# Soldann/MORB_SLAM

Measured on AMD Instinct MI355X. Metric: stereo frames/sec ORB extract+match (752x480, 1200 feat = BASELINE configs[1]), higher is better.
Workload: dtype u8; 1 GPU; BASELINE configs[1]: EuRoC-shaped stereo 752x480, 1200 feat: ORBextractor x2 + ComputeStereoMatches + ComputeBoW (synthetic k=10 L=6 vocabulary) + SearchByBoW vs previous frame; steps_in_flight=2, extract_streams=1, parallelism=frames dealt round-robin over 1 GPU(s)

## Files before the change

### morb_slam_amd/csrc/handles.h

```cpp
#pragma once
#include <cstdint>
#include <vector>

#include "common.h"
#include "hip_owned.h"

struct morb_matcher {
  int device = 0;
  morb::Stream stream;
  morb::DeviceGrow sortA;
  morb::DeviceGrow bin;
  morb::DeviceGrow sad;
  morb::DeviceGrow stereoRec;
  morb::DeviceGrow candKeys;
  morb::DeviceGrow candCount;
  morb::DeviceGrow evictJ;
  morb::DeviceGrow evictB;
  morb::DeviceGrow pairTables;
  morb::DeviceGrow newPointPairs;
  morb::DeviceGrow queries;
  morb::DeviceGrow queryCount;
  morb::DeviceGrow kfdbPair;
  morb::DeviceGrow kfdbList;
  morb::DeviceGrow scratch;
  struct ConstCopy { morb::DeviceArray<> d; std::vector<uint8_t> host; unsigned long long used = 0; };
  struct ConstSlot { ConstCopy way[4]; unsigned long long clock = 0; };
  enum ConstTable {
    kThresholdsPinhole = 0,
    kThresholdsKB8 = 1,
    kRigLastFrame = 2,
  };
  ConstSlot consts[4];
  std::vector<morb::DeviceArray<>> retired;
};

struct morb_optimizer {
  int device = 0;
  morb::Stream stream;
  morb::Stream side;
  morb::Event evFork, evJoin;
  morb::DeviceGrow work;
  morb::DeviceGrow spill;
  morb::DeviceGrow mlpnpCorr;
  morb::DeviceGrow twoViewCorr;
  morb::PinnedGrow stage;
  morb::PinnedArray<int> lmWords;
  int exactOrder = 1;
// ... 31 lines not shown
```

### morb_slam_amd/csrc/matcher.hip

```cpp
#include <hip/hip_runtime.h>

#include <algorithm>
#include <cstdlib>
#include <cstring>
#include <memory>
#include <vector>

#include "common.h"
#include "internal_abi.h"
#include "wave.h"
#include "extractor_internal.h"

using namespace morb;

namespace {

constexpr int TH_HIGH = 100, TH_LOW = 50, HISTO_LENGTH = 30;

struct Desc { uint32_t w[8]; };

__device__ __forceinline__ Desc load_desc(const uint8_t* p) {
  Desc d;
  const uint4* q = reinterpret_cast<const uint4*>(p);
  const uint4 a = q[0], b = q[1];
  d.w[0] = a.x; d.w[1] = a.y; d.w[2] = a.z; d.w[3] = a.w;
// ... 522 lines not shown
#pragma unroll
      for (int j = 0; j < CH; ++j) tc[j] = *reinterpret_cast<const uint2*>(nd + (size_t)min(cb + j, c0 + nc - 1) * 32);
#pragma unroll
      for (int j = 0; j < CH; ++j) {
        const int dd = quad_sum(__popc(d.x ^ tc[j].x) + __popc(d.y ^ tc[j].y));
        if (dd < bestd) { bestd = dd; best = min(cb + j, c0 + nc - 1); }
      }
    }
    final_id = best;
    if (level == nid_level) nid = final_id;
  } while (firstChild[final_id] >= 0);
  if (sub == 0) { wordId[o] = final_id; nodeId[o] = nid; }
}

__global__ __launch_bounds__(1024) void k_bow_sort(const int* __restrict__ node, const int* __restrict__ count, int cap,
                                                   int P, unsigned long long* __restrict__ sorted) {
  extern __shared__ unsigned long long skeys[];
  const int img = blockIdx.x, tid = threadIdx.x, NT = blockDim.x;
  const int n = count[img];
  if (n == 0) {
    for (int i = tid; i < cap; i += NT) sorted[(size_t)img * cap + i] = ~0ull;
    return;
  }
  for (int i = tid; i < P; i += NT) {
    unsigned long long k = ~0ull;
    if (i < n) {
      const int nd = node[(size_t)img * cap + i];
      if (nd >= 0) k = ((unsigned long long)(unsigned)nd << 32) | (unsigned)i;
    }
    skeys[i] = k;
  }
  __syncthreads();
  const bool onePass = P / 2 <= NT;
  for (int k = 2; k <= P; k <<= 1)
    for (int j = k >> 1; j > 0; j >>= 1) {
      for (int l = tid; l < P / 2; l += NT) {
        const int i = ((l & ~(j - 1)) << 1) | (l & (j - 1)), ixj = i | j;
        const unsigned long long a = skeys[i], b = skeys[ixj];
        const bool up = (i & k) == 0;
        if ((a > b) == up) { skeys[i] = b; skeys[ixj] = a; }
      }
      const int jn = j > 1 ? j >> 1 : k;
      if (onePass && jn < 64 && j < 64) { __builtin_amdgcn_fence(__ATOMIC_SEQ_CST, "wavefront"); __builtin_amdgcn_wave_barrier(); }
      else __syncthreads();
    }
  for (int i = tid; i < cap; i += NT) sorted[(size_t)img * cap + i] = i < P ? skeys[i] : ~0ull;
}

#ifdef MORB_FAST_TIMING
__device__ unsigned long long g_bowTrace[16384 * 4];
#define BOW_MARK(k) do { if (lane == 0 && bw_ < 16384) g_bowTrace[bw_ * 4 + (k)] = wall_clock64(); } while (0)
#else
#define BOW_MARK(k)
#endif
constexpr int BM_NB = 25;
constexpr int BM_FJ = 4;
__device__ __forceinline__ unsigned wave_min_u32(unsigned v) { return morbwave::min_u32(v); }
__global__ __launch_bounds__(256) void k_bow_match(const unsigned long long* __restrict__ sortedKF,
                                                   const unsigned long long* __restrict__ sortedF,
                                                   const int* __restrict__ nKFv, const int* __restrict__ nFv, int cap,
                                                   const uint8_t* __restrict__ descKF, const uint8_t* __restrict__ hasMP,
                                                   const morb_keypoint* __restrict__ kpsKF,
                                                   const uint8_t* __restrict__ descF, const morb_keypoint* __restrict__ kpsF,
                                                   const int* __restrict__ kfImg, const int* __restrict__ fImg,
                                                   float nnratio, int* __restrict__ matchF, int* __restrict__ binF,
                                                   const int* __restrict__ nLeftv,
                                                   const uint8_t* __restrict__ hasMP2, const int* __restrict__ nValidv,
                                                   int* __restrict__ matched2) {
  extern __shared__ __align__(16) unsigned long long bowLds[];
#ifdef MORB_FAST_TIMING
  const int bw_ = (blockIdx.y * gridDim.x + blockIdx.x) * 4 + (threadIdx.x >> 6);
  if ((threadIdx.x & 63) == 0 && bw_ < 16384) g_bowTrace[bw_ * 4] = wall_clock64();
#endif
  unsigned long long* sk = bowLds;
  unsigned long long* sf = bowLds + cap;
  const int pair = blockIdx.y, tid = threadIdx.x, lane = tid & 63, wv = tid >> 6;
  const int ik = kfImg[pair], jf = fImg[pair];
  const int nKF = nKFv[ik], nF = nFv[jf];
  const bool fish = nLeftv != nullptr && nLeftv[pair] >= 0;
  const int nLeft = fish ? nLeftv[pair] : 0x7fffffff;
  const bool kfkf = hasMP2 != nullptr;
  const int nValid1 = (kfkf && nValidv) ? nValidv[ik] : 0x7fffffff, nValid2 = (kfkf && nValidv) ? nValidv[jf] : 0x7fffffff;
  const int thLow = kfkf ? TH_LOW - 1 : TH_LOW;
  {
    const unsigned long long* gk = sortedKF + (size_t)ik * cap;
    const unsigned long long* gf = sortedF + (size_t)jf * cap;
    for (int i0 = 0; i0 < cap; i0 += 256 * 4) {
      unsigned long long a[4], b[4];
#pragma unroll
      for (int k = 0; k < 4; ++k) {
        const int i = i0 + k * 256 + tid;
        a[k] = i < nKF ? gk[i] : ~0ull;
        b[k] = i < nF ? gf[i] : ~0ull;
      }
#pragma unroll
      for (int k = 0; k < 4; ++k) {
        const int i = i0 + k * 256 + tid;
        if (i < nKF) sk[i] = a[k];
        if (i < nF) sf[i] = b[k];
      }
    }
  }
  __syncthreads();
  BOW_MARK(1);
  uint16_t* starts = reinterpret_cast<uint16_t*>(sf + cap);
  __shared__ int wcnt[4];
  const uint64_t ltm = lane == 0 ? 0ull : (~0ull >> (64 - lane));
  int nStarts = 0;
  for (int i0 = 0; i0 < nKF; i0 += 256) {
    const int i = i0 + tid;
    bool st = false;
    if (i < nKF) {
      const unsigned long long k = sk[i];
      st = k != ~0ull && (i == 0 || (unsigned)(sk[i - 1] >> 32) != (unsigned)(k >> 32));
    }
    const uint64_t m = __ballot(st);
    if (lane == 0) wcnt[wv] = __popcll(m);
    __syncthreads();
    int off = nStarts;
    for (int w = 0; w < wv; ++w) off += wcnt[w];
    if (st) starts[off + __popcll(m & ltm)] = (uint16_t)i;
    nStarts += wcnt[0] + wcnt[1] + wcnt[2] + wcnt[3];
    __syncthreads();
  }
  const int G = gridDim.x * 4, g = blockIdx.x * 4 + wv;
  BOW_MARK(2);
  int* mF = matchF + (size_t)pair * cap;
  int* bF = binF + (size_t)pair * cap;
  const float factor = 1.0f / HISTO_LENGTH;
  for (int o = g; o < nStarts; o += G) {
    const int p = starts[o];
    const unsigned node = (unsigned)(sk[p] >> 32);
    int lo = 0, hi = nF;
    const unsigned long long target = (unsigned long long)node << 32;
    while (lo < hi) {
      const int mid = (lo + hi) >> 1;
      if (sf[mid] < target) lo = mid + 1; else hi = mid;
    }
    const int fBeg = lo;
    int nFs = 0;
    bool more = false;
#pragma unroll
    for (int j = 0; j < BM_FJ; ++j) {
      const int s = fBeg + j * 64 + lane;
      const uint64_t mm = __ballot(s < nF && (unsigned)(sf[s] >> 32) == node);
      nFs += __popcll(mm);
      more = mm == ~0ull;
      if (mm != ~0ull) break;
    }
    if (nFs == 0) continue;
    if (!more) {
      const int nJ = (nFs + 63) >> 6;
      int idxF[BM_FJ], myMatch[BM_FJ], myBin[BM_FJ];
      Desc dF[BM_FJ];
      float angF[BM_FJ];
#pragma unroll
      for (int j = 0; j < BM_FJ; ++j) {
        idxF[j] = 0; myMatch[j] = -1; myBin[j] = 0; angF[j] = 0.f; dF[j] = Desc{};
        if (j < nJ && j * 64 + lane < nFs) {
          idxF[j] = (int)(sf[fBeg + j * 64 + lane] & 0xFFFFFFFFu);
          dF[j] = load_desc(descF + ((size_t)jf * cap + idxF[j]) * 32);
          angF[j] = kpsF[(size_t)jf * cap + idxF[j]].angle;
          if (kfkf && (!hasMP2[(size_t)jf * cap + idxF[j]] || idxF[j] >= nValid2)) myMatch[j] = -2;
        }
      }
      for (int q0 = p; q0 < nKF; q0 += 64) {
        const uint64_t mK = __ballot(q0 + lane < nKF && (unsigned)(sk[q0 + lane] >> 32) == node);
        const int nKs = mK == ~0ull ? 64 : (int)__builtin_ctzll(~mK);
        if (nKs == 0) break;
        int idxK = 0, has = 0;
        Desc dK = {};
        float angK = 0.f;
        if (lane < nKs) {
          idxK = (int)(sk[q0 + lane] & 0xFFFFFFFFu);
          has = hasMP[(size_t)ik * cap + idxK] && idxK < nValid1;
          dK = load_desc(descKF + ((size_t)ik * cap + idxK) * 32);
          angK = kpsKF[(size_t)ik * cap + idxK].angle;
        }
        for (int q = 0; q < nKs; ++q) {
          if (!__builtin_amdgcn_readlane(has, q)) continue;
          Desc dk;
#pragma unroll
          for (int w = 0; w < 8; ++w) dk.w[w] = (uint32_t)__builtin_amdgcn_readlane((int)dK.w[w], q);
          unsigned a1 = ~0u, a2 = ~0u;
          unsigned b1 = ~0u;
#pragma unroll
          for (int j = 0; j < BM_FJ; ++j)
            if (j < nJ && j * 64 + lane < nFs && myMatch[j] == -1) {
              const unsigned key = ((unsigned)hamming(dk, dF[j]) << 16) | (unsigned)idxF[j];
              if (idxF[j] < nLeft) { if (key < a1) { a2 = a1; a1 = key; } else if (key < a2) a2 = key; }
              else if (key < b1) b1 = key;
            }
          const unsigned k1 = wave_min_u32(a1);
          const unsigned k2 = wave_min_u32(a1 == k1 ? a2 : a1);
          const unsigned r1 = fish ? wave_min_u32(b1) : ~0u;
          const int bestDist1 = k1 == ~0u ? 256 : (int)(k1 >> 16);
          const int bestDist2 = k2 == ~0u ? 256 : (int)(k2 >> 16);
          const int bestDist1R = r1 == ~0u ? 256 : (int)(r1 >> 16);
          if (bestDist1 <= thLow) {
            const int realIdxKF = __builtin_amdgcn_readlane(idxK, q);
            const float aK = __int_as_float(__builtin_amdgcn_readlane(__float_as_int(angK), q));
            const bool takeL = (float)bestDist1 < nnratio * (float)bestDist2;
            const bool takeR = bestDist1R <= TH_LOW;
            const int wantIdx = (takeL && a1 == k1) ? (int)(k1 & 0xFFFFu) : -1;
            const int wantIdxR = (takeR && b1 == r1 && r1 != ~0u) ? (int)(r1 & 0xFFFFu) : -1;
#pragma unroll
            for (int j = 0; j < BM_FJ; ++j)
              if (j < nJ && j * 64 + lane < nFs && myMatch[j] == -1 && (idxF[j] == wantIdx || idxF[j] == wantIdxR)) {
                float rot = aK - angF[j];
                if (rot < 0.0f) rot += 360.0f;
                int bin = (int)roundf(rot * factor);
                if (bin == HISTO_LENGTH) bin = 0;
                myMatch[j] = realIdxKF; myBin[j] = bin;
              }
          }
        }
        if (nKs < 64) break;
      }
#pragma unroll
      for (int j = 0; j < BM_FJ; ++j)
        if (j < nJ && j * 64 + lane < nFs && myMatch[j] >= 0) {
          if (kfkf) { mF[myMatch[j]] = idxF[j]; bF[myMatch[j]] = myBin[j]; }
          else { mF[idxF[j]] = myMatch[j]; bF[idxF[j]] = myBin[j]; }
        }
      continue;
    }
    int fEnd = fBeg;
    while (fEnd < nF && (unsigned)(sf[fEnd] >> 32) == node) ++fEnd;
    for (int q = p; q < nKF; ++q) {
      const unsigned long long kq = sk[q];
      if (kq == ~0ull || (unsigned)(kq >> 32) != node) break;
      const int realIdxKF = (int)(kq & 0xFFFFFFFFu);
      if (!hasMP[(size_t)ik * cap + realIdxKF] || realIdxKF >= nValid1) continue;
      const Desc dKF = load_desc(descKF + ((size_t)ik * cap + realIdxKF) * 32);
      unsigned long long k1 = ~0ull, k2 = ~0ull, r1 = ~0ull, r2 = ~0ull;
      for (int s0 = fBeg; s0 < fEnd; s0 += 64) {
        const int s = s0 + lane;
        if (s < fEnd) {
          const int realIdxF = (int)(sf[s] & 0xFFFFFFFFu);
          const bool cand = kfkf ? (hasMP2[(size_t)jf * cap + realIdxF] && realIdxF < nValid2 && !matched2[(size_t)pair * cap + realIdxF])
                                 : (mF[realIdxF] < 0);
          if (cand) {
            const int d = hamming(dKF, load_desc(descF + ((size_t)jf * cap + realIdxF) * 32));
            const unsigned long long key = ((unsigned long long)d << 32) | (unsigned)realIdxF;
            const bool left = realIdxF < nLeft;
            unsigned long long t1 = left ? k1 : r1, t2 = left ? k2 : r2;
            top2_insert(t1, t2, key);
            k1 = left ? t1 : k1; k2 = left ? t2 : k2; r1 = left ? r1 : t1; r2 = left ? r2 : t2;
          }
        }
      }
      wave_top2(k1, k2);
      if (fish) wave_top2(r1, r2);
      const int bestDist1 = k1 == ~0ull ? 256 : (int)(k1 >> 32);
      const int bestDist2 = k2 == ~0ull ? 256 : (int)(k2 >> 32);
      const int bestDist1R = r1 == ~0ull ? 256 : (int)(r1 >> 32);
      if (bestDist1 <= thLow) {
        const float aK = kpsKF[(size_t)ik * cap + realIdxKF].angle;
        const bool takeL = (float)bestDist1 < nnratio * (float)bestDist2, takeR = bestDist1R <= TH_LOW;
        if (lane == 0) {
          if (takeL) {
            const int bestIdxF = (int)(k1 & 0xFFFFFFFFu);
            float rot = aK - kpsF[(size_t)jf * cap + bestIdxF].angle;
            if (rot < 0.0f) rot += 360.0f;
            int bin = (int)roundf(rot * factor);
            if (bin == HISTO_LENGTH) bin = 0;
            if (kfkf) { mF[realIdxKF] = bestIdxF; bF[realIdxKF] = bin; matched2[(size_t)pair * cap + bestIdxF] = 1; }
            else { mF[bestIdxF] = realIdxKF; bF[bestIdxF] = bin; }
          }
          if (takeR) {
            const int bestIdxFR = (int)(r1 & 0xFFFFFFFFu);
            float rot = aK - kpsF[(size_t)jf * cap + bestIdxFR].angle;
            if (rot < 0.0f) rot += 360.0f;
            int bin = (int)roundf(rot * factor);
            if (bin == HISTO_LENGTH) bin = 0;
            mF[bestIdxFR] = realIdxKF; bF[bestIdxFR] = bin;
          }
        }
        __builtin_amdgcn_fence(__ATOMIC_SEQ_CST, "workgroup");
        __builtin_amdgcn_wave_barrier();
      }
    }
  }
#ifdef MORB_FAST_TIMING
  BOW_MARK(3);
#endif
}

__global__ __launch_bounds__(64) void k_distinctive(const int* __restrict__ start, const uint8_t* __restrict__ desc,
                                                    int* __restrict__ bestIdx) {
  const int mp = blockIdx.x, lane = threadIdx.x;
  const int s0 = start[mp], N = start[mp + 1] - s0;
  if (N <= 0) { if (lane == 0) bestIdx[mp] = -1; return; }
  const uint8_t* D = desc + (size_t)s0 * 32;
  const int k = (N - 1) >> 1;
  unsigned best = ~0u;
  for (int i0 = 0; i0 < N; i0 += 64) {
// ... 17 lines not shown
}

__device__ void three_maxima(const int* cnt, int L, int& ind1, int& ind2, int& ind3) {
  int max1 = 0, max2 = 0, max3 = 0;
  ind1 = ind2 = ind3 = -1;
  for (int i = 0; i < L; i++) {
    const int s = cnt[i];
    if (s > max1) { max3 = max2; max2 = max1; max1 = s; ind3 = ind2; ind2 = ind1; ind1 = i; }
    else if (s > max2) { max3 = max2; max2 = s; ind3 = ind2; ind2 = i; }
    else if (s > max3) { max3 = s; ind3 = i; }
  }
  if (max2 < 0.1f * (float)max1) { ind2 = -1; ind3 = -1; }
  else if (max3 < 0.1f * (float)max1) { ind3 = -1; }
}

__global__ __launch_bounds__(256) void k_rot_filter(const int* __restrict__ nFv, const int* __restrict__ fImg, int cap,
                                                    int checkOri, int* __restrict__ matchF, const int* __restrict__ binF,
                                                    int* __restrict__ nmatches) {
  __shared__ int hist[HISTO_LENGTH];
  __shared__ int keep[3];
  __shared__ int total;
  const int pair = blockIdx.x, tid = threadIdx.x;
  const int nF = nFv[fImg[pair]];
  int* mF = matchF + (size_t)pair * cap;
  const int* bF = binF + (size_t)pair * cap;
  if (tid < HISTO_LENGTH) hist[tid] = 0;
  if (tid == 0) total = 0;
  __syncthreads();
  for (int i = tid; i < nF; i += 256)
    if (mF[i] >= 0) { atomicAdd(&total, 1); if (checkOri) atomicAdd(&hist[bF[i]], 1); }
  __syncthreads();
  if (checkOri) {
    if (tid == 0) three_maxima(hist, HISTO_LENGTH, keep[0], keep[1], keep[2]);
    __syncthreads();
    for (int i = tid; i < nF; i += 256)
      if (mF[i] >= 0) {
        const int b = bF[i];
        if (b != keep[0] && b != keep[1] && b != keep[2]) { mF[i] = -1; atomicSub(&total, 1); }
      }
    __syncthreads();
  }
  if (tid == 0) nmatches[pair] = total;
}

__global__ void k_fill_i32(int* p, size_t n, int v) {
  const size_t i = (size_t)blockIdx.x * 256 + threadIdx.x;
  if (i < n) p[i] = v;
}

}

extern "C" {

int morb_matcher_create(morb_matcher** out, int device) {
  MORB_REQUIRE(out, MORB_ERR_INVALID, "out is NULL");
  *out = nullptr;
  int ndev = 0;
// ... 35 lines not shown
    if (c.way[w].used < c.way[victim].used) victim = w;
  }
  morb_matcher::ConstCopy& k = c.way[victim];
  morb::DeviceArray<> fresh;
  MORB_HIP_CHECK(fresh.alloc(bytes));
  if (k.d) m->retired.push_back(std::move(k.d));
  k.d = std::move(fresh);
  k.host.assign((const uint8_t*)host, (const uint8_t*)host + bytes);
  k.used = ++c.clock;
  hipStream_t st = stream_or_own(m, stream);
  MORB_HIP_CHECK(hipMemcpyAsync(k.d, k.host.data(), bytes, hipMemcpyHostToDevice, st));
  MORB_HIP_CHECK(hipStreamSynchronize(st));
  *d_out = k.d;
  return MORB_OK;
}
int morb_bow_sort_images(morb_matcher* m, int nimg, const int* d_node, const int* d_count, int cap, unsigned long long** d_sorted,
                         void* stream) {
  int P = 1;
  while (P < cap) P <<= 1;
  MORB_REQUIRE((size_t)P * 8 <= 160 * 1024, MORB_ERR_UNSUPPORTED, "too many features per frame for the LDS sort");
  hipStream_t st = stream_or_own(m, stream);
  unsigned long long* sortA = nullptr;
  int rc = grow(m->sortA, (size_t)nimg * cap, &sortA);
  if (rc != MORB_OK) return rc;
  MORB_HIP_CHECK(hipFuncSetAttribute(reinterpret_cast<const void*>(k_bow_sort), hipFuncAttributeMaxDynamicSharedMemorySize, P * 8));
  hipLaunchKernelGGL(k_bow_sort, dim3(nimg), dim3(P / 2 < 64 ? 64 : P / 2 > 1024 ? 1024 : P / 2), (size_t)P * 8, st, d_node, d_count, cap, P, sortA);
  *d_sorted = sortA;
  return MORB_OK;
}

size_t morb_feature_slab_bytes(int S, int cap) {
  if (S <= 0 || cap <= 0) return 0;
  return (size_t)S * cap * (sizeof(morb_keypoint) + 32 + sizeof(int)) + (size_t)S * sizeof(int);
}
namespace {
__global__ __launch_bounds__(256) void k_slab_copy(int S, int cap, const int* __restrict__ rowIdx, uint32_t* kps, uint32_t* desc, uint32_t* node, int* count,
                                                   uint32_t* slab, int dir) {
  const int f = blockIdx.x, which = blockIdx.y;
  const int row = rowIdx ? rowIdx[f] : f;
  const size_t wK = (size_t)cap * 7, wD = (size_t)cap * 8, wN = (size_t)cap;
  uint32_t* sK = slab; uint32_t* sD = sK + (size_t)S * wK; uint32_t* sN = sD + (size_t)S * wD; uint32_t* sC = sN + (size_t)S * wN;
// ... 192 lines not shown
  MORB_REQUIRE(v, MORB_ERR_INVALID, "NULL vocabulary");
  if (weight) memcpy(weight, v->weight.data(), v->weight.size() * sizeof(double));
  if (scoring) *scoring = v->scoring;
  if (weighting) *weighting = v->weighting;
  return MORB_OK;
}

static int search_by_bow_impl(morb_matcher* m, int npairs, const int* d_kfImg, const int* d_fImg, int nimg,
                              const morb_keypoint* d_kps, const uint8_t* d_desc, const int* d_node, const int* d_count,
                              const uint8_t* d_hasMP, int cap, float nnratio, int checkOri, int* d_matchF,
                              int* d_nmatches, const int* d_nLeft, void* stream, const uint8_t* d_hasMP2 = nullptr,
                              const int* d_nValid = nullptr) {
  MORB_REQUIRE(m && d_kfImg && d_fImg && d_kps && d_desc && d_node && d_count && d_hasMP && d_matchF && d_nmatches,
               MORB_ERR_INVALID, "NULL argument");
  MORB_REQUIRE(npairs > 0 && nimg > 0 && cap > 0, MORB_ERR_INVALID, "bad sizes");
  int P = 1;
  while (P < cap) P <<= 1;
  MORB_REQUIRE((size_t)P * 8 <= 160 * 1024, MORB_ERR_UNSUPPORTED, "too many features per frame for the LDS sort");
  MORB_ENTER(st, m, stream);
  unsigned long long* sortA = nullptr;
  int* bin = nullptr;
  int rc = grow(m->sortA, (size_t)nimg * cap, &sortA);
  if (rc != MORB_OK) return rc;
  rc = grow(m->bin, (size_t)npairs * cap, &bin);
  if (rc != MORB_OK) return rc;
  MORB_HIP_CHECK(hipFuncSetAttribute(reinterpret_cast<const void*>(k_bow_sort), hipFuncAttributeMaxDynamicSharedMemorySize, P * 8));
  hipLaunchKernelGGL(k_bow_sort, dim3(nimg), dim3(P / 2 < 64 ? 64 : P / 2 > 1024 ? 1024 : P / 2), (size_t)P * 8, st, d_node, d_count, cap, P, sortA);
  const size_t nm = (size_t)npairs * cap;
  hipLaunchKernelGGL(k_fill_i32, dim3((unsigned)((nm + 255) / 256)), dim3(256), 0, st, d_matchF, nm, -1);
  int* matched2 = nullptr;
  if (d_hasMP2) {
    rc = grow(m->scratch, nm, &matched2);
    if (rc != MORB_OK) return rc;
    hipLaunchKernelGGL(k_fill_i32, dim3((unsigned)((nm + 255) / 256)), dim3(256), 0, st, matched2, nm, 0);
  }
  MORB_REQUIRE(cap < 65536 && (size_t)cap * 18 <= 160 * 1024, MORB_ERR_UNSUPPORTED, "too many features per frame for the LDS-resident node tables");
  MORB_HIP_CHECK(hipFuncSetAttribute(reinterpret_cast<const void*>(k_bow_match), hipFuncAttributeMaxDynamicSharedMemorySize, (int)((size_t)cap * 18)));
  hipLaunchKernelGGL(k_bow_match, dim3(BM_NB, npairs), dim3(256), (size_t)cap * 18, st, sortA, sortA, d_count, d_count,
                     cap, d_desc, d_hasMP, d_kps, d_desc, d_kps, d_kfImg, d_fImg, nnratio, d_matchF, bin, d_nLeft, d_hasMP2,
                     d_nValid, matched2);
  hipLaunchKernelGGL(k_rot_filter, dim3(npairs), dim3(256), 0, st, d_count, d_hasMP2 ? d_kfImg : d_fImg, cap, checkOri, d_matchF,
                     bin, d_nmatches);
  MORB_HIP_CHECK(hipGetLastError());
  return MORB_OK;
}

int morb_search_by_bow_batch(morb_matcher* m, int npairs, const int* d_kfImg, const int* d_fImg, int nimg,
                             const morb_keypoint* d_kps, const uint8_t* d_desc, const int* d_node, const int* d_count,
                             const uint8_t* d_hasMP, int cap, float nnratio, int checkOri, int* d_matchF,
                             int* d_nmatches, void* stream) {
  return search_by_bow_impl(m, npairs, d_kfImg, d_fImg, nimg, d_kps, d_desc, d_node, d_count, d_hasMP, cap, nnratio, checkOri,
                            d_matchF, d_nmatches, nullptr, stream);
}
// ... 37 lines not shown
```

Before: 140,100 frames/s.

## Precompute BoW node segments in sort kernel and add per-pair match kernel

The BoW sort kernel now also emits per-image segment tables (node id, first index, length), so the match kernel no longer rebuilds segment starts in every block of every pair. A new single-block-per-pair match kernel with LDS-resident 16-bit index tables, dynamic segment dealing and a fused rotation filter is added, but it is only chosen when npairs is at least 256 or an env var forces it. The change also caches the dynamic-LDS attribute calls and stops padding the sorted arrays out to cap. The cost is an extra segment pass inside the sort kernel and more code paths to keep correct.

```diff
diff --git a/morb_slam_amd/csrc/bow_segments.h b/morb_slam_amd/csrc/bow_segments.h
--- /dev/null
+++ b/morb_slam_amd/csrc/bow_segments.h
@@ -0,0 +1,50 @@
+#pragma once
+#include <cstdint>
+
+#if defined(__HIPCC__)
+#define BOWSEG_HD __host__ __device__ __forceinline__
+#else
+#define BOWSEG_HD inline
+#endif
+
+namespace morbseg {
+
+constexpr unsigned long long NO_WORD = ~0ull;
+
+BOWSEG_HD bool segment_starts(const unsigned long long* keys, int i) {
+  const unsigned long long k = keys[i];
+  return k != NO_WORD && (i == 0 || (uint32_t)(keys[i - 1] >> 32) != (uint32_t)(k >> 32));
+}
+
+BOWSEG_HD void segment_entry(const unsigned long long* keys, int n, int first, uint32_t* node, uint32_t* range) {
+  const uint32_t nd = (uint32_t)(keys[first] >> 32);
+  const unsigned long long last = ((unsigned long long)nd << 32) | 0xFFFFFFFFull;
+  int lo = first + 1, hi = n;
+  while (lo < hi) {
+    const int mid = (lo + hi) >> 1;
+    if (keys[mid] <= last) lo = mid + 1; else hi = mid;
+  }
+  *node = nd;
+  *range = (uint32_t)first | ((uint32_t)(lo - first) << 16);
+}
+
+BOWSEG_HD int segment_first(uint32_t range) { return (int)(range & 0xFFFFu); }
+BOWSEG_HD int segment_length(uint32_t range) { return (int)(range >> 16); }
+
+BOWSEG_HD int segment_find(const uint32_t* table, int nSeg, uint32_t node) {
+  int lo = 0, hi = nSeg;
+  while (lo < hi) {
+    const int mid = (lo + hi) >> 1;
+    if (table[2 * mid] < node) lo = mid + 1; else hi = mid;
+  }
+  return lo < nSeg && table[2 * lo] == node ? lo : -1;
+}
+
+inline int bow_segments_serial(const unsigned long long* keys, int n, uint32_t* table) {
+  int nSeg = 0;
+  for (int i = 0; i < n; ++i)
+    if (segment_starts(keys, i)) { segment_entry(keys, n, i, &table[2 * nSeg], &table[2 * nSeg + 1]); ++nSeg; }
+  return nSeg;
+}
+
+}
diff --git a/morb_slam_amd/csrc/handles.h b/morb_slam_amd/csrc/handles.h
--- a/morb_slam_amd/csrc/handles.h
+++ b/morb_slam_amd/csrc/handles.h
@@ -9,6 +9,7 @@
   int device = 0;
   morb::Stream stream;
   morb::DeviceGrow sortA;
+  morb::DeviceGrow bowSeg;
   morb::DeviceGrow bin;
   morb::DeviceGrow sad;
   morb::DeviceGrow stereoRec;
@@ -31,6 +32,7 @@
     kRigLastFrame = 2,
   };
   ConstSlot consts[4];
+  int bowSortLds = 0, bowMatchLds = 0, bowPairLds = 0;
   std::vector<morb::DeviceArray<>> retired;
 };
 
diff --git a/morb_slam_amd/csrc/matcher.hip b/morb_slam_amd/csrc/matcher.hip
--- a/morb_slam_amd/csrc/matcher.hip
+++ b/morb_slam_amd/csrc/matcher.hip
@@ -9,6 +9,7 @@
 #include "common.h"
 #include "internal_abi.h"
 #include "wave.h"
+#include "bow_segments.h"
 #include "extractor_internal.h"
 
 using namespace morb;
@@ -561,12 +562,14 @@
 }
 
 __global__ __launch_bounds__(1024) void k_bow_sort(const int* __restrict__ node, const int* __restrict__ count, int cap,
-                                                   int P, unsigned long long* __restrict__ sorted) {
+                                                   int P, unsigned long long* __restrict__ sorted,
+                                                   uint2* __restrict__ seg, int* __restrict__ segCount) {
   extern __shared__ unsigned long long skeys[];
+  __shared__ int wcnt[16];
   const int img = blockIdx.x, tid = threadIdx.x, NT = blockDim.x;
-  const int n = count[img];
-  if (n == 0) {
-    for (int i = tid; i < cap; i += NT) sorted[(size_t)img * cap + i] = ~0ull;
+  const int n = min(count[img], cap);
+  if (n <= 0) {
+    if (segCount && tid == 0) segCount[img] = 0;
     return;
   }
   for (int i = tid; i < P; i += NT) {
@@ -591,7 +594,30 @@
       if (onePass && jn < 64 && j < 64) { __builtin_amdgcn_fence(__ATOMIC_SEQ_CST, "wavefront"); __builtin_amdgcn_wave_barrier(); }
       else __syncthreads();
     }
-  for (int i = tid; i < cap; i += NT) sorted[(size_t)img * cap + i] = i < P ? skeys[i] : ~0ull;
+  __syncthreads();
+  for (int i = tid; i < n; i += NT) sorted[(size_t)img * cap + i] = skeys[i];
+  if (!seg) return;
+  const int lane = tid & 63, wv = tid >> 6, nW = NT >> 6;
+  const uint64_t ltm = lane == 0 ? 0ull : (~0ull >> (64 - lane));
+  uint2* sg = seg + (size_t)img * cap;
+  int nSeg = 0;
+  for (int i0 = 0; i0 < n; i0 += NT) {
+    const int i = i0 + tid;
+    const bool st = i < n && morbseg::segment_starts(skeys, i);
+    const uint64_t m = __ballot(st);
+    if (lane == 0) wcnt[wv] = __popcll(m);
+    __syncthreads();
+    int off = nSeg, all = 0;
+    for (int w = 0; w < nW; ++w) { const int c = wcnt[w]; all += c; off += w < wv ? c : 0; }
+    if (st) {
+      uint2 e;
+      morbseg::segment_entry(skeys, n, i, &e.x, &e.y);
+      sg[off + __popcll(m & ltm)] = e;
+    }
+    nSeg += all;
+    __syncthreads();
+  }
+  if (tid == 0) segCount[img] = nSeg;
 }
 
 #ifdef MORB_FAST_TIMING
@@ -602,9 +628,190 @@
 #endif
 constexpr int BM_NB = 25;
 constexpr int BM_FJ = 4;
+#ifndef MORB_BM_PAIR_WAVES
+#define MORB_BM_PAIR_WAVES 8
+#endif
+constexpr int BM_PAIR_WAVES = MORB_BM_PAIR_WAVES;
+constexpr int BM_PAIR_LONG = 16;
+constexpr int BM_PAIR_FROM = 256;
+constexpr int BM_PAIR_LDS = 13;
 __device__ __forceinline__ unsigned wave_min_u32(unsigned v) { return morbwave::min_u32(v); }
+
+struct BowPair {
+  int pair, ik, jf, cap, nKF, nF, nLeft, nValid1, nValid2, thLow;
+  bool fish, kfkf;
+  float nnratio;
+  const uint8_t* descKF; const uint8_t* hasMP; const morb_keypoint* kpsKF;
+  const uint8_t* descF; const morb_keypoint* kpsF; const uint8_t* hasMP2;
+  int* mF;
+  int* matched2;
+};
+__device__ __forceinline__ BowPair bow_pair(int pair, const int* __restrict__ nKFv, const int* __restrict__ nFv, int cap,
+                                            const uint8_t* descKF, const uint8_t* hasMP, const morb_keypoint* kpsKF,
+                                            const uint8_t* descF, const morb_keypoint* kpsF, const int* __restrict__ kfImg,
+                                            const int* __restrict__ fImg, float nnratio, int* matchF, const int* __restrict__ nLeftv,
+                                            const uint8_t* hasMP2, const int* __restrict__ nValidv, int* matched2) {
+  BowPair c;
+  c.pair = pair; c.cap = cap; c.nnratio = nnratio;
+  c.ik = kfImg[pair]; c.jf = fImg[pair];
+  c.nKF = min(nKFv[c.ik], cap); c.nF = min(nFv[c.jf], cap);
+  c.fish = nLeftv != nullptr && nLeftv[pair] >= 0;
+  c.nLeft = c.fish ? nLeftv[pair] : 0x7fffffff;
+  c.kfkf = hasMP2 != nullptr;
+  c.nValid1 = (c.kfkf && nValidv) ? nValidv[c.ik] : 0x7fffffff;
+  c.nValid2 = (c.kfkf && nValidv) ? nValidv[c.jf] : 0x7fffffff;
+  c.thLow = c.kfkf ? TH_LOW - 1 : TH_LOW;
+  c.descKF = descKF; c.hasMP = hasMP; c.kpsKF = kpsKF; c.descF = descF; c.kpsF = kpsF; c.hasMP2 = hasMP2;
+  c.mF = matchF + (size_t)pair * cap;
+  c.matched2 = matched2 ? matched2 + (size_t)pair * cap : nullptr;
+  return c;
+}
+
+struct SortedKeys { const unsigned long long* k; __device__ __forceinline__ int idx(int i) const { return (int)(k[i] & 0xFFFFFFFFu); } };
+struct SortedIdx16 { const uint16_t* k; __device__ __forceinline__ int idx(int i) const { return (int)k[i]; } };
+
+template <typename BinT, typename ListK, typename ListF>
+__device__ __forceinline__ void bow_match_node(const BowPair& c, const ListK sk, const ListF sf, const int p, const int nKseg,
+                                               const int fBeg, const int nFs, BinT* bF) {
+  const int lane = threadIdx.x & 63;
+  const int ik = c.ik, jf = c.jf, cap = c.cap, nLeft = c.nLeft, nValid1 = c.nValid1, nValid2 = c.nValid2, thLow = c.thLow;
+  const bool fish = c.fish, kfkf = c.kfkf;
+  const float nnratio = c.nnratio;
+  const uint8_t* descKF = c.descKF; const uint8_t* hasMP = c.hasMP; const uint8_t* descF = c.descF; const uint8_t* hasMP2 = c.hasMP2;
+  const morb_keypoint* kpsKF = c.kpsKF; const morb_keypoint* kpsF = c.kpsF;
+  int* mF = c.mF;
+  const float factor = 1.0f / HISTO_LENGTH;
+  if (nFs <= BM_FJ * 64) {
+    const int nJ = (nFs + 63) >> 6;
+    int idxF[BM_FJ], myMatch[BM_FJ], myBin[BM_FJ];
+    Desc dF[BM_FJ];
+    float angF[BM_FJ];
+#pragma unroll
+    for (int j = 0; j < BM_FJ; ++j) {
+      idxF[j] = 0; myMatch[j] = -1; myBin[j] = 0; angF[j] = 0.f; dF[j] = Desc{};
+      if (j < nJ && j * 64 + lane < nFs) {
+        idxF[j] = sf.idx(fBeg + j * 64 + lane);
+        dF[j] = load_desc(descF + ((size_t)jf * cap + idxF[j]) * 32);
+        angF[j] = kpsF[(size_t)jf * cap + idxF[j]].angle;
+        if (kfkf && (!hasMP2[(size_t)jf * cap + idxF[j]] || idxF[j] >= nValid2)) myMatch[j] = -2;
+      }
+    }
+    for (int q0 = p; q0 < p + nKseg; q0 += 64) {
+      const int nKs = min(64, p + nKseg - q0);
+      int idxK = 0, has = 0;
+      Desc dK = {};
+      float angK = 0.f;
+      if (lane < nKs) {
+        idxK = sk.idx(q0 + lane);
+        has = hasMP[(size_t)ik * cap + idxK] && idxK < nValid1;
+        dK = load_desc(descKF + ((size_t)ik * cap + idxK) * 32);
+        angK = kpsKF[(size_t)ik * cap + idxK].angle;
+      }
+      for (int q = 0; q < nKs; ++q) {
+        if (!__builtin_amdgcn_readlane(has, q)) continue;
+        Desc dk;
+#pragma unroll
+        for (int w = 0; w < 8; ++w) dk.w[w] = (uint32_t)__builtin_amdgcn_readlane((int)dK.w[w], q);
+        unsigned a1 = ~0u, a2 = ~0u;
+        unsigned b1 = ~0u;
+#pragma unroll
+        for (int j = 0; j < BM_FJ; ++j)
+          if (j < nJ && j * 64 + lane < nFs && myMatch[j] == -1) {
+            const unsigned key = ((unsigned)hamming(dk, dF[j]) << 16) | (unsigned)idxF[j];
+            if (idxF[j] < nLeft) { if (key < a1) { a2 = a1; a1 = key; } else if (key < a2) a2 = key; }
+            else if (key < b1) b1 = key;
+          }
+        const unsigned k1 = wave_min_u32(a1);
+        const unsigned k2 = wave_min_u32(a1 == k1 ? a2 : a1);
+        const unsigned r1 = fish ? wave_min_u32(b1) : ~0u;
+        const int bestDist1 = k1 == ~0u ? 256 : (int)(k1 >> 16);
+        const int bestDist2 = k2 == ~0u ? 256 : (int)(k2 >> 16);
+        const int bestDist1R = r1 == ~0u ? 256 : (int)(r1 >> 16);
+        if (bestDist1 <= thLow) {
+          const int realIdxKF = __builtin_amdgcn_readlane(idxK, q);
+          const float aK = __int_as_float(__builtin_amdgcn_readlane(__float_as_int(angK), q));
+          const bool takeL = (float)bestDist1 < nnratio * (float)bestDist2;
+          const bool takeR = bestDist1R <= TH_LOW;
+          const int wantIdx = (takeL && a1 == k1) ? (int)(k1 & 0xFFFFu) : -1;
+          const int wantIdxR = (takeR && b1 == r1 && r1 != ~0u) ? (int)(r1 & 0xFFFFu) : -1;
+#pragma unroll
+          for (int j = 0; j < BM_FJ; ++j)
+            if (j < nJ && j * 64 + lane < nFs && myMatch[j] == -1 && (idxF[j] == wantIdx || idxF[j] == wantIdxR)) {
+              float rot = aK - angF[j];
+              if (rot < 0.0f) rot += 360.0f;
+              int bin = (int)roundf(rot * factor);
+              if (bin == HISTO_LENGTH) bin = 0;
+              myMatch[j] = realIdxKF; myBin[j] = bin;
+            }
+        }
+      }
+    }
+#pragma unroll
+    for (int j = 0; j < BM_FJ; ++j)
+      if (j < nJ && j * 64 + lane < nFs && myMatch[j] >= 0) {
+        if (kfkf) { mF[myMatch[j]] = idxF[j]; bF[myMatch[j]] = (BinT)myBin[j]; }
+        else { mF[idxF[j]] = myMatch[j]; bF[idxF[j]] = (BinT)myBin[j]; }
+      }
+    return;
+  }
+  const int fEnd = fBeg + nFs;
+  for (int q = p; q < p + nKseg; ++q) {
+    const int realIdxKF = sk.idx(q);
+    if (!hasMP[(size_t)ik * cap + realIdxKF] || realIdxKF >= nValid1) continue;
+    const Desc dKF = load_desc(descKF + ((size_t)ik * cap + realIdxKF) * 32);
+    unsigned long long k1 = ~0ull, k2 = ~0ull, r1 = ~0ull, r2 = ~0ull;
+    for (int s0 = fBeg; s0 < fEnd; s0 += 64) {
+      const int s = s0 + lane;
+      if (s < fEnd) {
+        const int realIdxF = sf.idx(s);
+        const bool cand = kfkf ? (hasMP2[(size_t)jf * cap + realIdxF] && realIdxF < nValid2 && !c.matched2[realIdxF])
+                               : (mF[realIdxF] < 0);
+        if (cand) {
+          const int d = hamming(dKF, load_desc(descF + ((size_t)jf * cap + realIdxF) * 32));
+          const unsigned long long key = ((unsigned long long)d << 32) | (unsigned)realIdxF;
+          const bool left = realIdxF < nLeft;
+          unsigned long long t1 = left ? k1 : r1, t2 = left ? k2 : r2;
+          top2_insert(t1, t2, key);
+          k1 = left ? t1 : k1; k2 = left ? t2 : k2; r1 = left ? r1 : t1; r2 = left ? r2 : t2;
+        }
+      }
+    }
+    wave_top2(k1, k2);
+    if (fish) wave_top2(r1, r2);
+    const int bestDist1 = k1 == ~0ull ? 256 : (int)(k1 >> 32);
+    const int bestDist2 = k2 == ~0ull ? 256 : (int)(k2 >> 32);
+    const int bestDist1R = r1 == ~0ull ? 256 : (int)(r1 >> 32);
+    if (bestDist1 <= thLow) {
+      const float aK = kpsKF[(size_t)ik * cap + realIdxKF].angle;
+      const bool takeL = (float)bestDist1 < nnratio * (float)bestDist2, takeR = bestDist1R <= TH_LOW;
+      if (lane == 0) {
+        if (takeL) {
+          const int bestIdxF = (int)(k1 & 0xFFFFFFFFu);
+          float rot = aK - kpsF[(size_t)jf * cap + bestIdxF].angle;
+          if (rot < 0.0f) rot += 360.0f;
+          int bin = (int)roundf(rot * factor);
+          if (bin == HISTO_LENGTH) bin = 0;
+          if (kfkf) { mF[realIdxKF] = bestIdxF; bF[realIdxKF] = (BinT)bin; c.matched2[bestIdxF] = 1; }
+          else { mF[bestIdxF] = realIdxKF; bF[bestIdxF] = (BinT)bin; }
+        }
+        if (takeR) {
+          const int bestIdxFR = (int)(r1 & 0xFFFFFFFFu);
+          float rot = aK - kpsF[(size_t)jf * cap + bestIdxFR].angle;
+          if (rot < 0.0f) rot += 360.0f;
+          int bin = (int)roundf(rot * factor);
+          if (bin == HISTO_LENGTH) bin = 0;
+          mF[bestIdxFR] = realIdxKF; bF[bestIdxFR] = (BinT)bin;
+        }
+      }
+      __builtin_amdgcn_fence(__ATOMIC_SEQ_CST, "workgroup");
+      __builtin_amdgcn_wave_barrier();
+    }
+  }
+}
+
 __global__ __launch_bounds__(256) void k_bow_match(const unsigned long long* __restrict__ sortedKF,
                                                    const unsigned long long* __restrict__ sortedF,
+                                                   const uint2* __restrict__ seg, const int* __restrict__ segCount,
                                                    const int* __restrict__ nKFv, const int* __restrict__ nFv, int cap,
                                                    const uint8_t* __restrict__ descKF, const uint8_t* __restrict__ hasMP,
                                                    const morb_keypoint* __restrict__ kpsKF,
@@ -622,16 +829,12 @@
   unsigned long long* sk = bowLds;
   unsigned long long* sf = bowLds + cap;
   const int pair = blockIdx.y, tid = threadIdx.x, lane = tid & 63, wv = tid >> 6;
-  const int ik = kfImg[pair], jf = fImg[pair];
-  const int nKF = nKFv[ik], nF = nFv[jf];
-  const bool fish = nLeftv != nullptr && nLeftv[pair] >= 0;
-  const int nLeft = fish ? nLeftv[pair] : 0x7fffffff;
-  const bool kfkf = hasMP2 != nullptr;
-  const int nValid1 = (kfkf && nValidv) ? nValidv[ik] : 0x7fffffff, nValid2 = (kfkf && nValidv) ? nValidv[jf] : 0x7fffffff;
-  const int thLow = kfkf ? TH_LOW - 1 : TH_LOW;
+  const BowPair c = bow_pair(pair, nKFv, nFv, cap, descKF, hasMP, kpsKF, descF, kpsF, kfImg, fImg, nnratio, matchF, nLeftv, hasMP2,
+                             nValidv, matched2);
+  const int nKF = c.nKF, nF = c.nF;
   {
-    const unsigned long long* gk = sortedKF + (size_t)ik * cap;
-    const unsigned long long* gf = sortedF + (size_t)jf * cap;
+    const unsigned long long* gk = sortedKF + (size_t)c.ik * cap;
+    const unsigned long long* gf = sortedF + (size_t)c.jf * cap;
     for (int i0 = 0; i0 < cap; i0 += 256 * 4) {
       unsigned long long a[4], b[4];
 #pragma unroll
@@ -650,34 +853,15 @@
   }
   __syncthreads();
   BOW_MARK(1);
-  uint16_t* starts = reinterpret_cast<uint16_t*>(sf + cap);
-  __shared__ int wcnt[4];
-  const uint64_t ltm = lane == 0 ? 0ull : (~0ull >> (64 - lane));
-  int nStarts = 0;
-  for (int i0 = 0; i0 < nKF; i0 += 256) {
-    const int i = i0 + tid;
-    bool st = false;
-    if (i < nKF) {
-      const unsigned long long k = sk[i];
-      st = k != ~0ull && (i == 0 || (unsigned)(sk[i - 1] >> 32) != (unsigned)(k >> 32));
-    }
-    const uint64_t m = __ballot(st);
-    if (lane == 0) wcnt[wv] = __popcll(m);
-    __syncthreads();
-    int off = nStarts;
-    for (int w = 0; w < wv; ++w) off += wcnt[w];
-    if (st) starts[off + __popcll(m & ltm)] = (uint16_t)i;
-    nStarts += wcnt[0] + wcnt[1] + wcnt[2] + wcnt[3];
-    __syncthreads();
-  }
+  const uint2* segK = seg + (size_t)c.ik * cap;
+  const int nStarts = segCount[c.ik];
   const int G = gridDim.x * 4, g = blockIdx.x * 4 + wv;
   BOW_MARK(2);
-  int* mF = matchF + (size_t)pair * cap;
   int* bF = binF + (size_t)pair * cap;
-  const float factor = 1.0f / HISTO_LENGTH;
   for (int o = g; o < nStarts; o += G) {
-    const int p = starts[o];
-    const unsigned node = (unsigned)(sk[p] >> 32);
+    const uint2 e = segK[o];
+    const unsigned node = e.x;
+    const int p = morbseg::segment_first(e.y);
     int lo = 0, hi = nF;
     const unsigned long long target = (unsigned long long)node << 32;
     while (lo < hi) {
@@ -696,138 +880,12 @@
       if (mm != ~0ull) break;
     }
     if (nFs == 0) continue;
-    if (!more) {
-      const int nJ = (nFs + 63) >> 6;
-      int idxF[BM_FJ], myMatch[BM_FJ], myBin[BM_FJ];
-      Desc dF[BM_FJ];
-      float angF[BM_FJ];
-#pragma unroll
-      for (int j = 0; j < BM_FJ; ++j) {
-        idxF[j] = 0; myMatch[j] = -1; myBin[j] = 0; angF[j] = 0.f; dF[j] = Desc{};
-        if (j < nJ && j * 64 + lane < nFs) {
-          idxF[j] = (int)(sf[fBeg + j * 64 + lane] & 0xFFFFFFFFu);
-          dF[j] = load_desc(descF + ((size_t)jf * cap + idxF[j]) * 32);
-          angF[j] = kpsF[(size_t)jf * cap + idxF[j]].angle;
-          if (kfkf && (!hasMP2[(size_t)jf * cap + idxF[j]] || idxF[j] >= nValid2)) myMatch[j] = -2;
-        }
-      }
-      for (int q0 = p; q0 < nKF; q0 += 64) {
-        const uint64_t mK = __ballot(q0 + lane < nKF && (unsigned)(sk[q0 + lane] >> 32) == node);
-        const int nKs = mK == ~0ull ? 64 : (int)__builtin_ctzll(~mK);
-        if (nKs == 0) break;
-        int idxK = 0, has = 0;
-        Desc dK = {};
-        float angK = 0.f;
-        if (lane < nKs) {
-          idxK = (int)(sk[q0 + lane] & 0xFFFFFFFFu);
-          has = hasMP[(size_t)ik * cap + idxK] && idxK < nValid1;
-          dK = load_desc(descKF + ((size_t)ik * cap + idxK) * 32);
-          angK = kpsKF[(size_t)ik * cap + idxK].angle;
-        }
-        for (int q = 0; q < nKs; ++q) {
-          if (!__builtin_amdgcn_readlane(has, q)) continue;
-          Desc dk;
-#pragma unroll
-          for (int w = 0; w < 8; ++w) dk.w[w] = (uint32_t)__builtin_amdgcn_readlane((int)dK.w[w], q);
-          unsigned a1 = ~0u, a2 = ~0u;
-          unsigned b1 = ~0u;
-#pragma unroll
-          for (int j = 0; j < BM_FJ; ++j)
-            if (j < nJ && j * 64 + lane < nFs && myMatch[j] == -1) {
-              const unsigned key = ((unsigned)hamming(dk, dF[j]) << 16) | (unsigned)idxF[j];
-              if (idxF[j] < nLeft) { if (key < a1) { a2 = a1; a1 = key; } else if (key < a2) a2 = key; }
-              else if (key < b1) b1 = key;
-            }
-          const unsigned k1 = wave_min_u32(a1);
-          const unsigned k2 = wave_min_u32(a1 == k1 ? a2 : a1);
-          const unsigned r1 = fish ? wave_min_u32(b1) : ~0u;
-          const int bestDist1 = k1 == ~0u ? 256 : (int)(k1 >> 16);
-          const int bestDist2 = k2 == ~0u ? 256 : (int)(k2 >> 16);
-          const int bestDist1R = r1 == ~0u ? 256 : (int)(r1 >> 16);
-          if (bestDist1 <= thLow) {
-            const int realIdxKF = __builtin_amdgcn_readlane(idxK, q);
-            const float aK = __int_as_float(__builtin_amdgcn_readlane(__float_as_int(angK), q));
-            const bool takeL = (float)bestDist1 < nnratio * (float)bestDist2;
-            const bool takeR = bestDist1R <= TH_LOW;
-            const int wantIdx = (takeL && a1 == k1) ? (int)(k1 & 0xFFFFu) : -1;
-            const int wantIdxR = (takeR && b1 == r1 && r1 != ~0u) ? (int)(r1 & 0xFFFFu) : -1;
-#pragma unroll
-            for (int j = 0; j < BM_FJ; ++j)
-              if (j < nJ && j * 64 + lane < nFs && myMatch[j] == -1 && (idxF[j] == wantIdx || idxF[j] == wantIdxR)) {
-                float rot = aK - angF[j];
-                if (rot < 0.0f) rot += 360.0f;
-                int bin = (int)roundf(rot * factor);
-                if (bin == HISTO_LENGTH) bin = 0;
-                myMatch[j] = realIdxKF; myBin[j] = bin;
-              }
-          }
-        }
-        if (nKs < 64) break;
-      }
-#pragma unroll
-      for (int j = 0; j < BM_FJ; ++j)
-        if (j < nJ && j * 64 + lane < nFs && myMatch[j] >= 0) {
-          if (kfkf) { mF[myMatch[j]] = idxF[j]; bF[myMatch[j]] = myBin[j]; }
-          else { mF[idxF[j]] = myMatch[j]; bF[idxF[j]] = myBin[j]; }
-        }
-      continue;
-    }
-    int fEnd = fBeg;
-    while (fEnd < nF && (unsigned)(sf[fEnd] >> 32) == node) ++fEnd;
-    for (int q = p; q < nKF; ++q) {
-      const unsigned long long kq = sk[q];
-      if (kq == ~0ull || (unsigned)(kq >> 32) != node) break;
-      const int realIdxKF = (int)(kq & 0xFFFFFFFFu);
-      if (!hasMP[(size_t)ik * cap + realIdxKF] || realIdxKF >= nValid1) continue;
-      const Desc dKF = load_desc(descKF + ((size_t)ik * cap + realIdxKF) * 32);
-      unsigned long long k1 = ~0ull, k2 = ~0ull, r1 = ~0ull, r2 = ~0ull;
-      for (int s0 = fBeg; s0 < fEnd; s0 += 64) {
-        const int s = s0 + lane;
-        if (s < fEnd) {
-          const int realIdxF = (int)(sf[s] & 0xFFFFFFFFu);
-          const bool cand = kfkf ? (hasMP2[(size_t)jf * cap + realIdxF] && realIdxF < nValid2 && !matched2[(size_t)pair * cap + realIdxF])
-                                 : (mF[realIdxF] < 0);
-          if (cand) {
-            const int d = hamming(dKF, load_desc(descF + ((size_t)jf * cap + realIdxF) * 32));
-            const unsigned long long key = ((unsigned long long)d << 32) | (unsigned)realIdxF;
-            const bool left = realIdxF < nLeft;
-            unsigned long long t1 = left ? k1 : r1, t2 = left ? k2 : r2;
-            top2_insert(t1, t2, key);
-            k1 = left ? t1 : k1; k2 = left ? t2 : k2; r1 = left ? r1 : t1; r2 = left ? r2 : t2;
-          }
-        }
-      }
-      wave_top2(k1, k2);
-      if (fish) wave_top2(r1, r2);
-      const int bestDist1 = k1 == ~0ull ? 256 : (int)(k1 >> 32);
-      const int bestDist2 = k2 == ~0ull ? 256 : (int)(k2 >> 32);
-      const int bestDist1R = r1 == ~0ull ? 256 : (int)(r1 >> 32);
-      if (bestDist1 <= thLow) {
-        const float aK = kpsKF[(size_t)ik * cap + realIdxKF].angle;
-        const bool takeL = (float)bestDist1 < nnratio * (float)bestDist2, takeR = bestDist1R <= TH_LOW;
-        if (lane == 0) {
-          if (takeL) {
-            const int bestIdxF = (int)(k1 & 0xFFFFFFFFu);
-            float rot = aK - kpsF[(size_t)jf * cap + bestIdxF].angle;
-            if (rot < 0.0f) rot += 360.0f;
-            int bin = (int)roundf(rot * factor);
-            if (bin == HISTO_LENGTH) bin = 0;
-            if (kfkf) { mF[realIdxKF] = bestIdxF; bF[realIdxKF] = bin; matched2[(size_t)pair * cap + bestIdxF] = 1; }
-            else { mF[bestIdxF] = realIdxKF; bF[bestIdxF] = bin; }
-          }
-          if (takeR) {
-            const int bestIdxFR = (int)(r1 & 0xFFFFFFFFu);
-            float rot = aK - kpsF[(size_t)jf * cap + bestIdxFR].angle;
-            if (rot < 0.0f) rot += 360.0f;
-            int bin = (int)roundf(rot * factor);
-            if (bin == HISTO_LENGTH) bin = 0;
-            mF[bestIdxFR] = realIdxKF; bF[bestIdxFR] = bin;
-          }
-        }
-        __builtin_amdgcn_fence(__ATOMIC_SEQ_CST, "workgroup");
-        __builtin_amdgcn_wave_barrier();
-      }
-    }
+    if (more) {
+      int fEnd = fBeg + nFs;
+      while (fEnd < nF && (unsigned)(sf[fEnd] >> 32) == node) ++fEnd;
+      nFs = fEnd - fBeg;
+    }
+    bow_match_node<int>(c, SortedKeys{sk}, SortedKeys{sf}, p, morbseg::segment_length(e.y), fBeg, nFs, bF);
   }
 #ifdef MORB_FAST_TIMING
   BOW_MARK(3);
@@ -875,33 +933,89 @@
   else if (max3 < 0.1f * (float)max1) { ind3 = -1; }
 }
 
-__global__ __launch_bounds__(256) void k_rot_filter(const int* __restrict__ nFv, const int* __restrict__ fImg, int cap,
-                                                    int checkOri, int* __restrict__ matchF, const int* __restrict__ binF,
-                                                    int* __restrict__ nmatches) {
+template <typename BinT>
+__device__ __forceinline__ void rot_filter_pair(int n, int checkOri, int* mF, const BinT* bF, int* nmatches) {
   __shared__ int hist[HISTO_LENGTH];
   __shared__ int keep[3];
   __shared__ int total;
-  const int pair = blockIdx.x, tid = threadIdx.x;
-  const int nF = nFv[fImg[pair]];
-  int* mF = matchF + (size_t)pair * cap;
-  const int* bF = binF + (size_t)pair * cap;
+  const int tid = threadIdx.x, NT = blockDim.x;
   if (tid < HISTO_LENGTH) hist[tid] = 0;
   if (tid == 0) total = 0;
   __syncthreads();
-  for (int i = tid; i < nF; i += 256)
+  for (int i = tid; i < n; i += NT)
     if (mF[i] >= 0) { atomicAdd(&total, 1); if (checkOri) atomicAdd(&hist[bF[i]], 1); }
   __syncthreads();
   if (checkOri) {
     if (tid == 0) three_maxima(hist, HISTO_LENGTH, keep[0], keep[1], keep[2]);
     __syncthreads();
-    for (int i = tid; i < nF; i += 256)
+    for (int i = tid; i < n; i += NT)
       if (mF[i] >= 0) {
         const int b = bF[i];
         if (b != keep[0] && b != keep[1] && b != keep[2]) { mF[i] = -1; atomicSub(&total, 1); }
       }
     __syncthreads();
   }
-  if (tid == 0) nmatches[pair] = total;
+  if (tid == 0) *nmatches = total;
+}
+
+__global__ __launch_bounds__(256) void k_rot_filter(const int* __restrict__ nFv, const int* __restrict__ fImg, int cap,
+                                                    int checkOri, int* __restrict__ matchF, const int* __restrict__ binF,
+                                                    int* __restrict__ nmatches) {
+  const int pair = blockIdx.x;
+  rot_filter_pair<int>(min(nFv[fImg[pair]], cap), checkOri, matchF + (size_t)pair * cap, binF + (size_t)pair * cap, nmatches + pair);
+}
+
+__global__ __launch_bounds__(64 * BM_PAIR_WAVES) void k_bow_match_pair(const unsigned long long* __restrict__ sorted,
+                                                   const uint2* __restrict__ seg, const int* __restrict__ segCount,
+                                                   const int* __restrict__ countv, int cap,
+                                                   const uint8_t* __restrict__ desc, const uint8_t* __restrict__ hasMP,
+                                                   const morb_keypoint* __restrict__ kps,
+                                                   const int* __restrict__ kfImg, const int* __restrict__ fImg,
+                                                   float nnratio, int checkOri, int* __restrict__ matchF, int* __restrict__ nmatches,
+                                                   const int* __restrict__ nLeftv, const uint8_t* __restrict__ hasMP2,
+                                                   const int* __restrict__ nValidv, int* __restrict__ matched2) {
+  extern __shared__ __align__(16) unsigned long long bowLds[];
+  __shared__ int nextSeg;
+  uint32_t* segF = reinterpret_cast<uint32_t*>(bowLds);
+  uint16_t* ixK = reinterpret_cast<uint16_t*>(bowLds + cap);
+  uint16_t* ixF = ixK + cap;
+  uint8_t* bF = reinterpret_cast<uint8_t*>(ixF + cap);
+  const int pair = blockIdx.x, tid = threadIdx.x, lane = tid & 63, NT = blockDim.x;
+  const BowPair c = bow_pair(pair, countv, countv, cap, desc, hasMP, kps, desc, kps, kfImg, fImg, nnratio, matchF, nLeftv, hasMP2,
+                             nValidv, matched2);
+  const int nSegK = segCount[c.ik], nSegF = segCount[c.jf];
+  const uint2* segK = seg + (size_t)c.ik * cap;
+  const unsigned long long* sk = sorted + (size_t)c.ik * cap;
+  const unsigned long long* sf = sorted + (size_t)c.jf * cap;
+  for (int i = tid; i < cap; i += NT) {
+    c.mF[i] = -1;
+    if (c.matched2) c.matched2[i] = 0;
+    if (i < c.nKF) ixK[i] = (uint16_t)sk[i];
+    if (i < c.nF) ixF[i] = (uint16_t)sf[i];
+  }
+  {
+    const uint2* g = seg + (size_t)c.jf * cap;
+    for (int i = tid; i < nSegF; i += NT) { const uint2 e = g[i]; segF[2 * i] = e.x; segF[2 * i + 1] = e.y; }
+  }
+  if (tid == 0) nextSeg = 0;
+  __syncthreads();
+  const int nDeal = 2 * nSegK;
+  for (;;) {
+    int o = 0;
+    if (lane == 0) o = atomicAdd(&nextSeg, 1);
+    o = __builtin_amdgcn_readfirstlane(o);
+    if (o >= nDeal) break;
+    const bool second = o >= nSegK;
+    const uint2 e = segK[second ? o - nSegK : o];
+    if ((morbseg::segment_length(e.y) < BM_PAIR_LONG) != second) continue;
+    const int f = morbseg::segment_find(segF, nSegF, e.x);
+    if (f < 0) continue;
+    const uint32_t rF = segF[2 * f + 1];
+    bow_match_node<uint8_t>(c, SortedIdx16{ixK}, SortedIdx16{ixF}, morbseg::segment_first(e.y), morbseg::segment_length(e.y),
+                            morbseg::segment_first(rF), morbseg::segment_length(rF), bF);
+  }
+  __syncthreads();
+  rot_filter_pair<uint8_t>(c.kfkf ? c.nKF : c.nF, checkOri, c.mF, bF, nmatches + pair);
 }
 
 __global__ void k_fill_i32(int* p, size_t n, int v) {
@@ -967,17 +1081,31 @@
   *d_out = k.d;
   return MORB_OK;
 }
-int morb_bow_sort_images(morb_matcher* m, int nimg, const int* d_node, const int* d_count, int cap, unsigned long long** d_sorted,
-                         void* stream) {
+static int allow_lds(const void* kernel, int* allowed, size_t need) {
+  if ((int)need <= *allowed) return MORB_OK;
+  MORB_HIP_CHECK(hipFuncSetAttribute(kernel, hipFuncAttributeMaxDynamicSharedMemorySize, (int)need));
+  *allowed = (int)need;
+  return MORB_OK;
+}
+static int launch_bow_sort(morb_matcher* m, hipStream_t st, int nimg, const int* d_node, const int* d_count, int cap,
+                           unsigned long long* sortA, uint2* seg, int* segCount) {
   int P = 1;
   while (P < cap) P <<= 1;
   MORB_REQUIRE((size_t)P * 8 <= 160 * 1024, MORB_ERR_UNSUPPORTED, "too many features per frame for the LDS sort");
+  const int rc = allow_lds(reinterpret_cast<const void*>(k_bow_sort), &m->bowSortLds, (size_t)P * 8);
+  if (rc != MORB_OK) return rc;
+  hipLaunchKernelGGL(k_bow_sort, dim3(nimg), dim3(P / 2 < 64 ? 64 : P / 2 > 1024 ? 1024 : P / 2), (size_t)P * 8, st, d_node, d_count, cap, P, sortA,
+                     seg, segCount);
+  return MORB_OK;
+}
+int morb_bow_sort_images(morb_matcher* m, int nimg, const int* d_node, const int* d_count, int cap, unsigned long long** d_sorted,
+                         void* stream) {
   hipStream_t st = stream_or_own(m, stream);
   unsigned long long* sortA = nullptr;
   int rc = grow(m->sortA, (size_t)nimg * cap, &sortA);
   if (rc != MORB_OK) return rc;
-  MORB_HIP_CHECK(hipFuncSetAttribute(reinterpret_cast<const void*>(k_bow_sort), hipFuncAttributeMaxDynamicSharedMemorySize, P * 8));
-  hipLaunchKernelGGL(k_bow_sort, dim3(nimg), dim3(P / 2 < 64 ? 64 : P / 2 > 1024 ? 1024 : P / 2), (size_t)P * 8, st, d_node, d_count, cap, P, sortA);
+  rc = launch_bow_sort(m, st, nimg, d_node, d_count, cap, sortA, nullptr, nullptr);
+  if (rc != MORB_OK) return rc;
   *d_sorted = sortA;
   return MORB_OK;
 }
@@ -1200,29 +1328,44 @@
   MORB_REQUIRE(m && d_kfImg && d_fImg && d_kps && d_desc && d_node && d_count && d_hasMP && d_matchF && d_nmatches,
                MORB_ERR_INVALID, "NULL argument");
   MORB_REQUIRE(npairs > 0 && nimg > 0 && cap > 0, MORB_ERR_INVALID, "bad sizes");
-  int P = 1;
-  while (P < cap) P <<= 1;
-  MORB_REQUIRE((size_t)P * 8 <= 160 * 1024, MORB_ERR_UNSUPPORTED, "too many features per frame for the LDS sort");
+  MORB_REQUIRE(cap < 65536, MORB_ERR_UNSUPPORTED, "too many features per frame for the 16-bit feature fields");
   MORB_ENTER(st, m, stream);
   unsigned long long* sortA = nullptr;
-  int* bin = nullptr;
+  uint2* seg = nullptr;
   int rc = grow(m->sortA, (size_t)nimg * cap, &sortA);
   if (rc != MORB_OK) return rc;
-  rc = grow(m->bin, (size_t)npairs * cap, &bin);
+  rc = grow(m->bowSeg, (size_t)nimg * cap + (size_t)(nimg + 1) / 2, &seg);
   if (rc != MORB_OK) return rc;
-  MORB_HIP_CHECK(hipFuncSetAttribute(reinterpret_cast<const void*>(k_bow_sort), hipFuncAttributeMaxDynamicSharedMemorySize, P * 8));
-  hipLaunchKernelGGL(k_bow_sort, dim3(nimg), dim3(P / 2 < 64 ? 64 : P / 2 > 1024 ? 1024 : P / 2), (size_t)P * 8, st, d_node, d_count, cap, P, sortA);
+  int* segCount = reinterpret_cast<int*>(seg + (size_t)nimg * cap);
+  rc = launch_bow_sort(m, st, nimg, d_node, d_count, cap, sortA, seg, segCount);
+  if (rc != MORB_OK) return rc;
   const size_t nm = (size_t)npairs * cap;
-  hipLaunchKernelGGL(k_fill_i32, dim3((unsigned)((nm + 255) / 256)), dim3(256), 0, st, d_matchF, nm, -1);
   int* matched2 = nullptr;
   if (d_hasMP2) {
     rc = grow(m->scratch, nm, &matched2);
     if (rc != MORB_OK) return rc;
-    hipLaunchKernelGGL(k_fill_i32, dim3((unsigned)((nm + 255) / 256)), dim3(256), 0, st, matched2, nm, 0);
-  }
-  MORB_REQUIRE(cap < 65536 && (size_t)cap * 18 <= 160 * 1024, MORB_ERR_UNSUPPORTED, "too many features per frame for the LDS-resident node tables");
-  MORB_HIP_CHECK(hipFuncSetAttribute(reinterpret_cast<const void*>(k_bow_match), hipFuncAttributeMaxDynamicSharedMemorySize, (int)((size_t)cap * 18)));
-  hipLaunchKernelGGL(k_bow_match, dim3(BM_NB, npairs), dim3(256), (size_t)cap * 18, st, sortA, sortA, d_count, d_count,
+  }
+  const char* form = getenv("MORB_BOW_FORM");
+  const bool forcePair = form && !strcmp(form, "pair"), forceNode = form && !strcmp(form, "node");
+  const size_t lds = (size_t)cap * BM_PAIR_LDS;
+  MORB_REQUIRE(!forcePair || lds <= 160 * 1024, MORB_ERR_UNSUPPORTED, "too many features per frame for the pair form's LDS tables");
+  if (lds <= 160 * 1024 && (forcePair || (!forceNode && npairs >= BM_PAIR_FROM))) {
+    rc = allow_lds(reinterpret_cast<const void*>(k_bow_match_pair), &m->bowPairLds, lds);
+    if (rc != MORB_OK) return rc;
+    hipLaunchKernelGGL(k_bow_match_pair, dim3(npairs), dim3(64 * BM_PAIR_WAVES), lds, st, sortA, seg, segCount, d_count, cap, d_desc, d_hasMP,
+                       d_kps, d_kfImg, d_fImg, nnratio, checkOri, d_matchF, d_nmatches, d_nLeft, d_hasMP2, d_nValid, matched2);
+    MORB_HIP_CHECK(hipGetLastError());
+    return MORB_OK;
+  }
+  int* bin = nullptr;
+  rc = grow(m->bin, nm, &bin);
+  if (rc != MORB_OK) return rc;
+  hipLaunchKernelGGL(k_fill_i32, dim3((unsigned)((nm + 255) / 256)), dim3(256), 0, st, d_matchF, nm, -1);
+  if (d_hasMP2) hipLaunchKernelGGL(k_fill_i32, dim3((unsigned)((nm + 255) / 256)), dim3(256), 0, st, matched2, nm, 0);
+  MORB_REQUIRE((size_t)cap * 16 <= 160 * 1024, MORB_ERR_UNSUPPORTED, "too many features per frame for the LDS-resident key tables");
+  rc = allow_lds(reinterpret_cast<const void*>(k_bow_match), &m->bowMatchLds, (size_t)cap * 16);
+  if (rc != MORB_OK) return rc;
+  hipLaunchKernelGGL(k_bow_match, dim3(BM_NB, npairs), dim3(256), (size_t)cap * 16, st, sortA, sortA, seg, segCount, d_count, d_count,
                      cap, d_desc, d_hasMP, d_kps, d_desc, d_kps, d_kfImg, d_fImg, nnratio, d_matchF, bin, d_nLeft, d_hasMP2,
                      d_nValid, matched2);
   hipLaunchKernelGGL(k_rot_filter, dim3(npairs), dim3(256), 0, st, d_count, d_hasMP2 ? d_kfImg : d_fImg, cap, checkOri, d_matchF,
```

Result: no change. 141,200 frames/s (median of 6 runs) (+0.8%).
